# wyhuai/DDNM

Hardware: AMD Instinct MI355X
Metric: restored images/sec @256×256, 100 DDIM steps, 4×SR; 1/2/4/8 GPU (higher is better)
Workload: dtype f32 (3x3 convolutions: fp32 operands carried as hi + lo fp16 halves, three fp16 MFMA products per product, fp32 accumulate -- operand error 2^-22, measured closer to fp64 than the fp32 MFMA kernel; everything else fp32); 1 GPU; celeba_hq.yml SVD sr_bicubic 4x, sigma_y=0, eta=0.85, T_sampling=100, batch_size=8 per GPU (BASELINE configs[1]); global_batch=8, image=3x256x256, parallelism=dp1 (image sharding)

## Files before the change

ddnm_amd/csrc/conv_s16_persist.hip:

```cpp
#include <type_traits>

#include "s16_tile.h"

namespace {
enum { K_MID = 0, K_LAST = 1, K_FIRST = 2 };

constexpr int p_spread(int tap) { return tap == 0 ? 10 : (tap <= 6 ? 9 : 0); }
constexpr int p_first_of(int tap) { return tap == 0 ? 0 : (tap <= 7 ? 10 + 9 * (tap - 1) : S16_NOUT); }
static_assert(p_first_of(7) == S16_NOUT, "64 values over taps 0..6");
constexpr int p_extra(int kind, int tap, bool has_res, bool ascale) {
    return kind == K_FIRST ? p_spread(tap) + (tap == 0 ? 1 : 0)
                           : (kind == K_LAST ? (tap == 0 ? 4 + (ascale ? 1 : 0) : 0) + (has_res ? p_spread(tap) : 0) : 0);
}
constexpr int p_base(int tap) {
    return (tap == 1 || tap == 2) ? S16_BR + S16_HSPLIT + 2 : ((tap == 4 || tap == 5) ? S16_BR + S16_HR - S16_HSPLIT : S16_BR);
}
constexpr int p_wait(int kind, int tap, bool has_res, bool ascale) {
    return p_base(tap) + (tap >= 1 ? p_extra(kind, tap - 1, has_res, ascale) : 0) + (tap >= 2 ? p_extra(kind, tap - 2, has_res, ascale) : 0);
}
static_assert(p_wait(K_FIRST, 2, true, true) < 64 && p_wait(K_LAST, 2, true, true) < 64, "vmcnt is a 6-bit field");

template <int V>
using ic = std::integral_constant<int, V>;

}

template <bool ASCALE, bool HAS_RES, bool HAS_SKIP = false>
__global__ __launch_bounds__(S16_NTHREADS, 1) void conv3x3_s16_persist_kernel(const ConvArgs p, const int total) {
    static_assert(!HAS_SKIP || (ASCALE && !HAS_RES), "a fused shortcut reads a raw operand (bound required) and replaces the residual");
    constexpr int WM = S16_WM, WN = S16_WN, MT = S16_MT, NT = S16_NT, BN = S16_BN, HR = S16_HR, HSPLIT = S16_HSPLIT, LDH = S16_LDH, KCH = S16_KCH;
    constexpr int MAXH = S16_MAXH, HWd = S16_HWD, NWB = S16_NWB, WTILE = S16_WTILE, BR = S16_BR, NTHREADS = S16_NTHREADS;
    __shared__ __attribute__((aligned(1024))) char lds_all[NWB * WTILE + S16_HBYTES + WM * BN * 2 * 4];
    char* const Bs = lds_all;
    _Float16* const Hs = reinterpret_cast<_Float16*>(lds_all + NWB * WTILE);
    float* const stat_lds = reinterpret_cast<float*>(lds_all + NWB * WTILE + S16_HBYTES);

    const ddnm_conv_desc& d = p.d;
    const int tid = threadIdx.x, lane = tid & 63;
    const int wave = __builtin_amdgcn_readfirstlane(tid >> 6);
    const int wm = wave / WN, wn = wave % WN;
    const int G = gridDim.x;
    const int per_img = (d.Ho * d.Wo) >> 8;
    const int Cout = d.Cout, Wo = d.Wo;

    int t_img, t_ty0, t_tx0, t_ntile, t_mtile;
    auto tile_of = [&](int v) {
        const int tile_id = xcd_swizzle(v, total);
        t_ntile = tile_id % p.n_tiles;
        t_mtile = tile_id / p.n_tiles;
        t_img = t_mtile / per_img;
        const int t = t_mtile - t_img * per_img;
        const int ty = t / p.tiles_x;
        t_ty0 = ty * 8;
        t_tx0 = (t - ty * p.tiles_x) * 32;
    };

    const int hc = tid % S16_HCOLS, prow = tid / S16_HCOLS;
    int hoff[HR];
    auto set_hoff = [&]() {
#pragma unroll
        for (int i = 0; i < HR; ++i) {
            const int row = prow + S16_HRPP * i;
            const int hy = row / HWd, hx = row - hy * HWd;
            const int iy = t_ty0 - 1 + hy, ix = t_tx0 - 1 + hx;
            const bool ok = row < MAXH && (unsigned)iy < (unsigned)d.Hin && (unsigned)ix < (unsigned)d.Win;
            const int sy = d.ups ? (iy >> 1) : iy, sx = d.ups ? (ix >> 1) : ix;
            hoff[i] = ok ? (t_img * p.Hs + sy) * p.Ws + sx : -1;
        }
    };

    const int lrow = lane >> 3, lpiece = lane & 7;
    const int wswz = S16_W_SWZ(wave, lrow);
    const unsigned w_rowlen = 9u * (unsigned)p.Cin * 4u;
    const __amdgpu_buffer_rsrc_t r_w = __builtin_amdgcn_make_buffer_rsrc(
        const_cast<void*>(reinterpret_cast<const void*>(d.weight)), 0, (unsigned)p.n_tiles * BN * w_rowlen, 0x00020000);
    const unsigned w_lane = S16_W_LANE(wave * 8 + lrow, w_rowlen, lpiece, wswz);
    unsigned w_soff = 0;
    auto issue_w = [&](int chunk, int tap, int buf) {
        s16_w_request<BR, NTHREADS / 64>(r_w, Bs + buf * WTILE + wave * 1024, w_lane, w_soff + ((unsigned)tap * p.Cin + (unsigned)chunk * KCH) * 4u, w_rowlen);
    };

    const int nchunks = p.Cin / KCH;
    uint4 h_st[HR];
    f32x4 gsc = {1.f, 1.f, 1.f, 1.f}, gsh = {0.f, 0.f, 0.f, 0.f};
    const bool has_gn = d.gn_scale != nullptr;
    constexpr unsigned HOOB = 0x80000000u;
    const __amdgpu_buffer_rsrc_t r_s0 = __builtin_amdgcn_make_buffer_rsrc(
        const_cast<void*>(reinterpret_cast<const void*>(d.src0)), 0, (unsigned)d.B * p.Hs * p.Ws * d.C0 * 4, 0x00020000);
    const __amdgpu_buffer_rsrc_t r_s1 = __builtin_amdgcn_make_buffer_rsrc(
        const_cast<void*>(reinterpret_cast<const void*>(d.C1 > 0 ? d.src1 : d.src0)), 0,
        (unsigned)d.B * p.Hs * p.Ws * (d.C1 > 0 ? d.C1 : d.C0) * 4, 0x00020000);
    const __amdgpu_buffer_rsrc_t r_amax = __builtin_amdgcn_make_buffer_rsrc(
        const_cast<void*>(reinterpret_cast<const void*>(d.amax_in)), 0, d.amax_in ? (unsigned)d.B * DDNM_AMAX_N * 4u : 0u, 0x00020000);
    unsigned amax_bits = 0;
    int gn_img = 0;
    float ascale_stage = 1.f;
    auto prefetch_halo_part = [&](int chunk, int i0, int i1, bool live = true) {
        const int cb = chunk * KCH;
        const bool first = cb < d.C0;
        const unsigned cs = first ? d.C0 : d.C1, coff = first ? cb : cb - d.C0;
        const __amdgpu_buffer_rsrc_t r_s = first ? r_s0 : r_s1;
#pragma unroll
        for (int i = 0; i < HR; ++i) {
            if (i < i0 || i >= i1) continue;
            const unsigned vo = (hoff[i] >= 0 && live) ? ((unsigned)hoff[i] * cs + hc * 4) * 4 : HOOB;
            const u32x4 v = __builtin_amdgcn_raw_buffer_load_b128(r_s, vo, coff * 4, 0);
            h_st[i] = uint4{v.x, v.y, v.z, v.w};
        }
        if (i0 == 0) {
            const float* gb = has_gn ? d.gn_scale + (size_t)gn_img * p.Cin + hc * 4 + cb : reinterpret_cast<const float*>(d.weight);
            const float* hb2 = has_gn ? d.gn_shift + (size_t)gn_img * p.Cin + hc * 4 + cb : reinterpret_cast<const float*>(d.weight);
            gsc = *reinterpret_cast<const f32x4*>(gb);
            gsh = *reinterpret_cast<const f32x4*>(hb2);
        }
    };
    auto stage_halo_part = [&](int hbuf, int i0, int i1) {
#pragma unroll
        for (int i = 0; i < HR; ++i) {
            if (i < i0 || i >= i1) continue;
            const int row = prow + S16_HRPP * i;
            if (row < MAXH) {
                _Float16* dst = &Hs[hbuf * MAXH * LDH + row * LDH + hc * 4];
                f32x4 v = __builtin_bit_cast(f32x4, h_st[i]);
                if (has_gn && hoff[i] >= 0) v = gn_act(v, gsc, gsh, d.gn_silu);
                if constexpr (ASCALE) split_store(dst, v, ascale_stage);
                else split_store(dst, v);
            }
        }
    };

    f32x16 acc[MT][NT];
#pragma unroll
    for (int i = 0; i < MT; ++i)
#pragma unroll
        for (int j = 0; j < NT; ++j)
#pragma unroll
            for (int r = 0; r < 16; ++r) acc[i][j][r] = 0.f;
    int a_off[MT];
#pragma unroll
    for (int i = 0; i < MT; ++i) {
        const int m = (wm * MT + i) * 32 + (lane & 31);
        a_off[i] = ((m >> 5) * HWd + (m & 31)) * LDH + (lane >> 5) * 8;
    }
    const int b_frag = S16_B_FRAG(wn * NT * 32, lane);
    auto mfma_tap = [&](int tap, int buf, int hbuf) {
        const int ky = tap / 3, kx = tap - 3 * ky;
        const int tap_off = (ky * HWd + kx) * LDH + hbuf * MAXH * LDH;
        s16_mfma_tile<MT, NT>(acc, Hs, a_off, tap_off, Bs + buf * WTILE, b_frag);
    };

    const int ncol = lane & 31, rsel = 4 * (lane >> 5);
    const unsigned out_bytes = (unsigned)d.B * d.Ho * Wo * Cout * 4u;
    const __amdgpu_buffer_rsrc_t r_out = __builtin_amdgcn_make_buffer_rsrc(reinterpret_cast<void*>(d.out), 0, out_bytes, 0x00020000);
    const __amdgpu_buffer_rsrc_t r_res = __builtin_amdgcn_make_buffer_rsrc(
        const_cast<void*>(reinterpret_cast<const void*>(d.res)), 0, d.res ? out_bytes : 0u, 0x00020000);
    const __amdgpu_buffer_rsrc_t r_bias = __builtin_amdgcn_make_buffer_rsrc(
        const_cast<void*>(reinterpret_cast<const void*>(d.bias)), 0, d.bias ? (unsigned)Cout * 4u : 0u, 0x00020000);
    const __amdgpu_buffer_rsrc_t r_badd = __builtin_amdgcn_make_buffer_rsrc(
        const_cast<void*>(reinterpret_cast<const void*>(d.badd)), 0,
        d.badd ? (unsigned)((d.B - 1) * d.badd_stride + Cout) * 4u : 0u, 0x00020000);
    const __amdgpu_buffer_rsrc_t r_stats = __builtin_amdgcn_make_buffer_rsrc(
        reinterpret_cast<void*>(d.stats_out), 0, d.stats_out ? (unsigned)p.m_tiles * Cout * 8u : 0u, 0x00020000);
    const unsigned o_lane = (unsigned)(((wm * MT * Wo + rsel) * Cout + wn * NT * 32 + ncol) * 4);
    auto o_soff = [&](unsigned base, int k) {
        const int i = k >> 5, j = (k >> 4) & 1, r = k & 15;
        return base + (unsigned)(((i * Wo + (r & 3) + 8 * (r >> 2)) * Cout + j * 32) * 4);
    };
    auto tile_base = [&]() { return (unsigned)((((t_img * d.Ho + t_ty0) * Wo + t_tx0) * Cout + t_ntile * BN) * 4); };
    const unsigned c_lane = (unsigned)((wn * NT * 32 + ncol) * 4);
    const unsigned st_lane = tid < 2 * BN ? (unsigned)(tid * 4) : HOOB;

    float outv[S16_NOUT];
    float addv[NT][2];
#pragma unroll
    for (int k = 0; k < S16_NOUT; ++k) outv[k] = 0.f;
#pragma unroll
    for (int j = 0; j < NT; ++j) addv[j][0] = addv[j][1] = 0.f;
    unsigned pend_base = 0, pend_stats = 0;
    unsigned cur_base = 0, cur_stats = 0;
    float epi_cur = d.acc_scale;

    auto finalize = [&]() {
        const float add[NT] = {addv[0][0], addv[1][0]};
        s16_tile_finalize<HAS_RES ? S16_RES_TILE : S16_RES_ZERO>(acc, outv, add, epi_cur, stat_lds, wm, wn, lane);
        pend_base = cur_base;
        pend_stats = cur_stats;
    };
    auto store_stats = [&]() {
        s16_store_stats(stat_lds, tid, r_stats, st_lane, pend_stats);
    };

    int v = blockIdx.x;
    tile_of(v);
    set_hoff();
    gn_img = t_img;
    w_soff = (unsigned)t_ntile * BN * w_rowlen;
    cur_base = tile_base();
    cur_stats = (unsigned)((t_mtile * Cout + t_ntile * BN) * 8);
    if constexpr (ASCALE) {
        float inv;
        s16_amax_scales(s16_amax_request(r_amax, lane, t_img, true), has_gn, ascale_stage, inv);
        epi_cur = d.acc_scale * inv;
    }
    prefetch_halo_part(0, 0, HR);
    issue_w(0, 0, 0);
    issue_w(0, 1, 1);
    stage_halo_part(0, 0, HR);
    if (wave >= WM * WN / 2) __builtin_amdgcn_s_setprio(1);

    int hb = 0, n_img_next = 0;
    bool have_next = false;
    float epi_next = epi_cur;
    unsigned next_base = 0, next_stats = 0, next_wsoff = 0;

    auto tap_body = [&](auto KIND, auto TAP, int chunk) {
        constexpr int kind = decltype(KIND)::value, tap = decltype(TAP)::value;
        constexpr int cur = tap % NWB;
        asm volatile("s_waitcnt vmcnt(%0) lgkmcnt(0)" ::"n"(p_wait(kind, tap, HAS_RES, ASCALE)) : "memory");
        __builtin_amdgcn_s_barrier();
        asm volatile("" ::: "memory");
        if constexpr (kind == K_LAST && tap >= 7) {
            if (tap == 7 && have_next) w_soff = next_wsoff;
            issue_w(0, tap - 7, cur >= 1 ? cur - 1 : NWB - 1);
        } else {
            issue_w(tap + 2 < 9 ? chunk : chunk + 1, (tap + 2) % 9, cur >= 1 ? cur - 1 : NWB - 1);
        }
        asm volatile("" ::: "memory");
        __builtin_amdgcn_sched_barrier(0);
        const int nchunk = kind == K_LAST ? 0 : chunk + 1;
        const bool live = kind == K_LAST ? have_next : true;
        if constexpr (tap == 0) prefetch_halo_part(nchunk, 0, HSPLIT, live);
        if constexpr (tap == 3) {
            if constexpr (kind == K_LAST && ASCALE) {
                if (have_next) {
                    float inv;
                    s16_amax_scales(amax_bits, has_gn, ascale_stage, inv);
                    epi_next = d.acc_scale * inv;
                }
            }
            if (live) stage_halo_part(hb ^ 1, 0, HSPLIT);
            prefetch_halo_part(nchunk, HSPLIT, HR, live);
        }
        if constexpr (tap == 6) {
            if (live) stage_halo_part(hb ^ 1, HSPLIT, HR);
        }
        asm volatile("" ::: "memory");
        __builtin_amdgcn_sched_barrier(0);
        if constexpr (kind == K_FIRST) {
            if constexpr (tap == 0) store_stats();
#pragma unroll
            for (int k = p_first_of(tap); k < p_first_of(tap + 1); ++k)
                __builtin_amdgcn_raw_buffer_store_b32(__float_as_uint(outv[k]), r_out, o_lane, o_soff(pend_base, k), 0);
        }
        if constexpr (kind == K_LAST) {
            if constexpr (tap == 0) {
                if constexpr (ASCALE) amax_bits = s16_amax_request(r_amax, lane, n_img_next, have_next);
#pragma unroll
                for (int j = 0; j < NT; ++j) {
                    addv[j][0] = __uint_as_float(__builtin_amdgcn_raw_buffer_load_b32(r_bias, c_lane + j * 128, (unsigned)(t_ntile * BN * 4), 0));
                    addv[j][1] = __uint_as_float(__builtin_amdgcn_raw_buffer_load_b32(r_badd, c_lane + j * 128, (unsigned)((t_img * d.badd_stride + t_ntile * BN) * 4), 0));
                }
            }
            if constexpr (tap == 4) {
#pragma unroll
                for (int j = 0; j < NT; ++j) addv[j][0] = addv[j][0] + addv[j][1];
            }
            if constexpr (HAS_RES) {
#pragma unroll
                for (int k = p_first_of(tap); k < p_first_of(tap + 1); ++k)
                    outv[k] = __uint_as_float(__builtin_amdgcn_raw_buffer_load_b32(r_res, o_lane, o_soff(cur_base, k), 0));
            }
        }
        asm volatile("" ::: "memory");
        __builtin_amdgcn_sched_barrier(0);
        mfma_tap(tap, cur, hb);
    };
    auto run_chunk = [&](auto KIND, int chunk) {
        tap_body(KIND, ic<0>{}, chunk);
        tap_body(KIND, ic<1>{}, chunk);
        tap_body(KIND, ic<2>{}, chunk);
        tap_body(KIND, ic<3>{}, chunk);
        tap_body(KIND, ic<4>{}, chunk);
        tap_body(KIND, ic<5>{}, chunk);
        tap_body(KIND, ic<6>{}, chunk);
        tap_body(KIND, ic<7>{}, chunk);
        tap_body(KIND, ic<8>{}, chunk);
        hb ^= 1;
    };

    constexpr int SR = 4;
    const int sc8 = tid & 7, srow = tid >> 3;
    int s_img = 0, s_ty0 = 0, s_tx0 = 0;
    f32x4 s_st[SR];
    const int SCin = d.SC0 + d.SC1;
    const unsigned sw_rowlen = (unsigned)SCin * 4u;
    const __amdgpu_buffer_rsrc_t r_sw = __builtin_amdgcn_make_buffer_rsrc(
        const_cast<void*>(reinterpret_cast<const void*>(d.skip_weight)), 0, HAS_SKIP ? (unsigned)p.n_tiles * BN * sw_rowlen : 0u, 0x00020000);
    const unsigned sw_lane = S16_W_LANE(wave * 8 + lrow, sw_rowlen, lpiece, wswz);
    unsigned sw_soff = 0;
    auto skip_setup = [&](int img, int ty0, int tx0, int ntile) {
        s_img = img;
        s_ty0 = ty0;
        s_tx0 = tx0;
        sw_soff = (unsigned)ntile * BN * sw_rowlen;
    };
    auto skip_prefetch = [&](int ch) {
        const int cb = ch * KCH;
        const float* src;
        int cs, coff;
        if (cb < d.SC0) { src = d.skip0; cs = d.SC0; coff = cb; }
        else { src = d.skip1; cs = d.SC1; coff = cb - d.SC0; }
#pragma unroll
        for (int i = 0; i < SR; ++i) {
            const int m = srow + 64 * i;
            const int so = (s_img * p.Hs + s_ty0 + (m >> 5)) * p.Ws + s_tx0 + (m & 31);
            s_st[i] = *reinterpret_cast<const f32x4*>(src + (size_t)so * cs + coff + sc8 * 4);
        }
    };
    auto skip_issue_w = [&](int ch) {
        s16_w_request<BR, NTHREADS / 64>(r_sw, Bs + 2 * WTILE + wave * 1024, sw_lane, sw_soff + (unsigned)ch * KCH * 4u, sw_rowlen);
    };
    auto skip_phase = [&](int hbuf, float ascale_cur, int img, int ty0, int tx0, int ntile) {
        const int nsk = SCin / KCH;
        skip_setup(img, ty0, tx0, ntile);
        skip_prefetch(0);
        for (int ch = 0; ch < nsk; ++ch) {
            __syncthreads();
            skip_issue_w(ch);
#pragma unroll
            for (int i = 0; i < SR; ++i) {
                const int m = srow + 64 * i;
                split_store(&Hs[hbuf * MAXH * LDH + (((m >> 5) + 1) * HWd + (m & 31) + 1) * LDH + sc8 * 4], s_st[i], ascale_cur);
            }
            asm volatile("s_waitcnt vmcnt(0)" ::: "memory");
            __syncthreads();
            if (ch + 1 < nsk) skip_prefetch(ch + 1);
            mfma_tap(4, 2, hbuf);
        }
    };

    bool pending = false;
    for (;;) {
        int c0 = 0;
        if (pending) {
            run_chunk(ic<K_FIRST>{}, 0);
            c0 = 1;
        }
        for (int chunk = c0; chunk < nchunks - 1; ++chunk) run_chunk(ic<K_MID>{}, chunk);
        const int vn = v + G;
        have_next = vn < total;
        const int c_img = t_img, c_ntile = t_ntile;
        const float ascale_cur = ascale_stage;
        const int c_ty0 = t_ty0, c_tx0 = t_tx0;
        if (have_next) {
            tile_of(vn);
            set_hoff();
            gn_img = t_img;
            next_wsoff = (unsigned)t_ntile * BN * w_rowlen;
            next_base = tile_base();
            next_stats = (unsigned)((t_mtile * Cout + t_ntile * BN) * 8);
            n_img_next = t_img;
        }
        {
            const int n_img = t_img, n_ntile = t_ntile;
            t_img = c_img;
            t_ntile = c_ntile;
            run_chunk(ic<K_LAST>{}, nchunks - 1);
            t_img = n_img;
            t_ntile = n_ntile;
        }
        if constexpr (HAS_SKIP) skip_phase(hb ^ 1, ascale_cur, c_img, c_ty0, c_tx0, c_ntile);
        finalize();
        if (!have_next) break;
        v = vn;
        cur_base = next_base;
        cur_stats = next_stats;
        epi_cur = epi_next;
        pending = true;
    }
    __syncthreads();
    store_stats();
#pragma unroll
    for (int k = 0; k < S16_NOUT; ++k) __builtin_amdgcn_raw_buffer_store_b32(__float_as_uint(outv[k]), r_out, o_lane, o_soff(pend_base, k), 0);
}

bool conv3x3_s16_persist_eligible(const ConvArgs& p) {
    const ddnm_conv_desc& d = p.d;
    const long tiles = (long)p.m_tiles * p.n_tiles;
    if (d.skip0 && (!d.amax_in || d.res)) return false;
    return p.ksplit == 1 && tiles >= 512 && p.TW == 32 && !d.res_ups && !d.out_nchw && p.Cin / S16_KCH >= 2 &&
           (int64_t)d.B * d.Ho * d.Wo * d.Cout * 4 < ((int64_t)1 << 31) && (int64_t)p.m_tiles * d.Cout * 8 < ((int64_t)1 << 31);
}

int conv3x3_s16_persist_launch(const ConvArgs& p, hipStream_t s) {
    const int cus = conv_persist_grid_cus();
    const int total = p.m_tiles * p.n_tiles;
    const dim3 grid(total < cus ? total : cus);
    const bool asc = p.d.amax_in != nullptr, res = p.d.res != nullptr;
    if (p.d.skip0) { DDNM_LAUNCH((conv3x3_s16_persist_kernel<true, false, true>), grid, dim3(S16_NTHREADS), 0, s, p, total); }
    else if (asc && res) { DDNM_LAUNCH((conv3x3_s16_persist_kernel<true, true>), grid, dim3(S16_NTHREADS), 0, s, p, total); }
    else if (asc) { DDNM_LAUNCH((conv3x3_s16_persist_kernel<true, false>), grid, dim3(S16_NTHREADS), 0, s, p, total); }
    else if (res) { DDNM_LAUNCH((conv3x3_s16_persist_kernel<false, true>), grid, dim3(S16_NTHREADS), 0, s, p, total); }
    else { DDNM_LAUNCH((conv3x3_s16_persist_kernel<false, false>), grid, dim3(S16_NTHREADS), 0, s, p, total); }
    return 0;
}
```

Measured before the change: 6.447 images/sec.

## Software-pipeline the skip 1x1 phase with double-buffered weights and activations

```diff
diff --git a/ddnm_amd/csrc/conv_s16_persist.hip b/ddnm_amd/csrc/conv_s16_persist.hip
--- a/ddnm_amd/csrc/conv_s16_persist.hip
+++ b/ddnm_amd/csrc/conv_s16_persist.hip
@@ -213,6 +213,43 @@
     float epi_next = epi_cur;
     unsigned next_base = 0, next_stats = 0, next_wsoff = 0;
 
+    constexpr int SR = 4;
+    const int sc8 = tid & 7, srow = tid >> 3;
+    int s_img = 0, s_ty0 = 0, s_tx0 = 0;
+    f32x4 s_st[2][SR];
+    const int SCin = d.SC0 + d.SC1;
+    const unsigned sw_rowlen = (unsigned)SCin * 4u;
+    const __amdgpu_buffer_rsrc_t r_sw = __builtin_amdgcn_make_buffer_rsrc(
+        const_cast<void*>(reinterpret_cast<const void*>(d.skip_weight)), 0, HAS_SKIP ? (unsigned)p.n_tiles * BN * sw_rowlen : 0u, 0x00020000);
+    const unsigned sw_lane = S16_W_LANE(wave * 8 + lrow, sw_rowlen, lpiece, wswz);
+    unsigned sw_soff = 0;
+    const __amdgpu_buffer_rsrc_t r_k0 = __builtin_amdgcn_make_buffer_rsrc(
+        const_cast<void*>(reinterpret_cast<const void*>(d.skip0)), 0, HAS_SKIP ? (unsigned)d.B * p.Hs * p.Ws * d.SC0 * 4 : 0u, 0x00020000);
+    const __amdgpu_buffer_rsrc_t r_k1 = __builtin_amdgcn_make_buffer_rsrc(
+        const_cast<void*>(reinterpret_cast<const void*>(d.SC1 > 0 ? d.skip1 : d.skip0)), 0,
+        HAS_SKIP ? (unsigned)d.B * p.Hs * p.Ws * (d.SC1 > 0 ? d.SC1 : d.SC0) * 4 : 0u, 0x00020000);
+    auto skip_setup = [&](int img, int ty0, int tx0, int ntile) {
+        s_img = img;
+        s_ty0 = ty0;
+        s_tx0 = tx0;
+        sw_soff = (unsigned)ntile * BN * sw_rowlen;
+    };
+    auto skip_prefetch = [&](int ch, auto SET) {
+        const int cb = ch * KCH;
+        const bool first = cb < d.SC0;
+        const unsigned cs = first ? d.SC0 : d.SC1, coff = first ? cb : cb - d.SC0;
+        const __amdgpu_buffer_rsrc_t r_k = first ? r_k0 : r_k1;
+#pragma unroll
+        for (int i = 0; i < SR; ++i) {
+            const int m = srow + 64 * i;
+            const unsigned so = (unsigned)((s_img * p.Hs + s_ty0 + (m >> 5)) * p.Ws + s_tx0 + (m & 31));
+            s_st[decltype(SET)::value][i] = __builtin_bit_cast(f32x4, __builtin_amdgcn_raw_buffer_load_b128(r_k, (so * cs + sc8 * 4) * 4, coff * 4, 0));
+        }
+    };
+    auto skip_issue_w = [&](int ch, int buf) {
+        s16_w_request<BR, NTHREADS / 64>(r_sw, Bs + buf * WTILE + wave * 1024, sw_lane, sw_soff + (unsigned)ch * KCH * 4u, sw_rowlen);
+    };
+
     auto tap_body = [&](auto KIND, auto TAP, int chunk) {
         constexpr int kind = decltype(KIND)::value, tap = decltype(TAP)::value;
         constexpr int cur = tap % NWB;
@@ -221,7 +258,17 @@
         asm volatile("" ::: "memory");
         if constexpr (kind == K_LAST && tap >= 7) {
             if (tap == 7 && have_next) w_soff = next_wsoff;
-            issue_w(0, tap - 7, cur >= 1 ? cur - 1 : NWB - 1);
+            if constexpr (HAS_SKIP && tap == 8) {
+                skip_prefetch(0, ic<0>{});
+                asm volatile("" ::: "memory");
+                __builtin_amdgcn_sched_barrier(0);
+                skip_issue_w(0, 1);
+                asm volatile("" ::: "memory");
+                __builtin_amdgcn_sched_barrier(0);
+                skip_prefetch(SCin > KCH ? 1 : 0, ic<1>{});
+            } else {
+                issue_w(0, tap - 7, cur >= 1 ? cur - 1 : NWB - 1);
+            }
         } else {
             issue_w(tap + 2 < 9 ? chunk : chunk + 1, (tap + 2) % 9, cur >= 1 ? cur - 1 : NWB - 1);
         }
@@ -288,55 +335,45 @@
         hb ^= 1;
     };
 
-    constexpr int SR = 4;
-    const int sc8 = tid & 7, srow = tid >> 3;
-    int s_img = 0, s_ty0 = 0, s_tx0 = 0;
-    f32x4 s_st[SR];
-    const int SCin = d.SC0 + d.SC1;
-    const unsigned sw_rowlen = (unsigned)SCin * 4u;
-    const __amdgpu_buffer_rsrc_t r_sw = __builtin_amdgcn_make_buffer_rsrc(
-        const_cast<void*>(reinterpret_cast<const void*>(d.skip_weight)), 0, HAS_SKIP ? (unsigned)p.n_tiles * BN * sw_rowlen : 0u, 0x00020000);
-    const unsigned sw_lane = S16_W_LANE(wave * 8 + lrow, sw_rowlen, lpiece, wswz);
-    unsigned sw_soff = 0;
-    auto skip_setup = [&](int img, int ty0, int tx0, int ntile) {
-        s_img = img;
-        s_ty0 = ty0;
-        s_tx0 = tx0;
-        sw_soff = (unsigned)ntile * BN * sw_rowlen;
-    };
-    auto skip_prefetch = [&](int ch) {
-        const int cb = ch * KCH;
-        const float* src;
-        int cs, coff;
-        if (cb < d.SC0) { src = d.skip0; cs = d.SC0; coff = cb; }
-        else { src = d.skip1; cs = d.SC1; coff = cb - d.SC0; }
-#pragma unroll
-        for (int i = 0; i < SR; ++i) {
-            const int m = srow + 64 * i;
-            const int so = (s_img * p.Hs + s_ty0 + (m >> 5)) * p.Ws + s_tx0 + (m & 31);
-            s_st[i] = *reinterpret_cast<const f32x4*>(src + (size_t)so * cs + coff + sc8 * 4);
-        }
-    };
-    auto skip_issue_w = [&](int ch) {
-        s16_w_request<BR, NTHREADS / 64>(r_sw, Bs + 2 * WTILE + wave * 1024, sw_lane, sw_soff + (unsigned)ch * KCH * 4u, sw_rowlen);
-    };
-    auto skip_phase = [&](int hbuf, float ascale_cur, int img, int ty0, int tx0, int ntile) {
+    auto skip_phase = [&](int hbuf, float ascale_cur) {
         const int nsk = SCin / KCH;
-        skip_setup(img, ty0, tx0, ntile);
-        skip_prefetch(0);
-        for (int ch = 0; ch < nsk; ++ch) {
-            __syncthreads();
-            skip_issue_w(ch);
+        auto skip_chunk = [&](auto BUF, auto TAIL, int ch) {
+            constexpr int buf = decltype(BUF)::value;
+            constexpr bool tail = decltype(TAIL)::value != 0;
+            const int nx = ch + 1 < nsk ? ch + 1 : ch, nx2 = ch + 2 < nsk ? ch + 2 : nsk - 1;
+            __builtin_amdgcn_sched_barrier(0);
+            asm volatile("s_waitcnt lgkmcnt(0)" ::: "memory");
+            __builtin_amdgcn_s_barrier();
+            asm volatile("" ::: "memory");
 #pragma unroll
             for (int i = 0; i < SR; ++i) {
                 const int m = srow + 64 * i;
-                split_store(&Hs[hbuf * MAXH * LDH + (((m >> 5) + 1) * HWd + (m & 31) + 1) * LDH + sc8 * 4], s_st[i], ascale_cur);
-            }
-            asm volatile("s_waitcnt vmcnt(0)" ::: "memory");
-            __syncthreads();
-            if (ch + 1 < nsk) skip_prefetch(ch + 1);
-            mfma_tap(4, 2, hbuf);
-        }
+                split_store(&Hs[hbuf * MAXH * LDH + (((m >> 5) + 1) * HWd + (m & 31) + 1) * LDH + sc8 * 4], s_st[buf - 1][i], ascale_cur);
+            }
+            asm volatile("" ::: "memory");
+            __builtin_amdgcn_sched_barrier(0);
+            skip_issue_w(nx, 3 - buf);
+            asm volatile("" ::: "memory");
+            __builtin_amdgcn_sched_barrier(0);
+            if constexpr (!tail) skip_prefetch(nx2, ic<buf - 1>{});
+            asm volatile("s_waitcnt vmcnt(%0) lgkmcnt(0)" ::"n"(tail ? SR + BR : 2 * SR + BR) : "memory");
+            __builtin_amdgcn_s_barrier();
+            asm volatile("" ::: "memory");
+            mfma_tap(4, buf, hbuf);
+        };
+        int ch = 0;
+        for (; ch + 1 < nsk; ch += 2) {
+            skip_chunk(ic<1>{}, ic<0>{}, ch);
+            skip_chunk(ic<2>{}, ic<0>{}, ch + 1);
+        }
+        if (ch < nsk) skip_chunk(ic<1>{}, ic<1>{}, ch);
+        asm volatile("s_waitcnt lgkmcnt(0)" ::: "memory");
+        __builtin_amdgcn_s_barrier();
+        asm volatile("" ::: "memory");
+        skip_issue_w(nsk - 1, 2);
+        issue_w(0, 1, 1);
+        asm volatile("" ::: "memory");
+        __builtin_amdgcn_sched_barrier(0);
     };
 
     bool pending = false;
@@ -365,11 +402,12 @@
             const int n_img = t_img, n_ntile = t_ntile;
             t_img = c_img;
             t_ntile = c_ntile;
+            if constexpr (HAS_SKIP) skip_setup(c_img, c_ty0, c_tx0, c_ntile);
             run_chunk(ic<K_LAST>{}, nchunks - 1);
             t_img = n_img;
             t_ntile = n_ntile;
         }
-        if constexpr (HAS_SKIP) skip_phase(hb ^ 1, ascale_cur, c_img, c_ty0, c_tx0, c_ntile);
+        if constexpr (HAS_SKIP) skip_phase(hb ^ 1, ascale_cur);
         finalize();
         if (!have_next) break;
         v = vn;
```

New measurement: 6.464 images/sec, median of 6. Within noise of the previous version (+0.3%).
